# falfab/orb_slam_cuda

Measured on AMD Instinct MI355X. Metric: frames/s ORB extract+match, 1241×376 mono nFeatures=2000; achieved HBM GB/s, higher is better.
Workload: dtype u8

## Files before the change

orb_slam_cuda_amd/csrc/orbx_blur.hip:

```cpp
#include "orbx_device.cuh"

namespace orbx {

#ifndef ORBX_BLUR_TH
#define ORBX_BLUR_TH 48
#endif
#ifndef ORBX_BLUR_TW
#define ORBX_BLUR_TW 128
#endif
constexpr int kBlurTWs = 64, kBlurTHs = 32;

typedef unsigned short us2_t __attribute__((ext_vector_type(2)));
__device__ __forceinline__ uint32_t dot4(uint32_t px, uint32_t taps, uint32_t acc) {
  return __builtin_amdgcn_udot4(px, taps, acc, false);
}
__device__ __forceinline__ uint32_t dot2(uint32_t pair, uint32_t taps, uint32_t acc) {
  return __builtin_amdgcn_udot2(__builtin_bit_cast(us2_t, pair), __builtin_bit_cast(us2_t, taps), acc, false);
}

template <int kBlurTW, int kBlurTH>
__global__ __launch_bounds__(256) void blur_kernel(ExtractParams P, LevelPtrs lp, const int2* __restrict__ rtab,
                                                   int tiles, int ntiles, unsigned magic, uint8_t* __restrict__ blur) {
  constexpr int kBlurInW = kBlurTW + 32;
  constexpr int kBlurPairs = (kBlurTH + 6 + 1) / 2;
  __shared__ __attribute__((aligned(16))) uint8_t in[kBlurPairs * 2][kBlurInW];
  __shared__ __attribute__((aligned(16))) uint32_t tmp[kBlurPairs][kBlurTW];
  const int wg = xcd_remap(blockIdx.x + blockIdx.y * gridDim.x, gridDim.x * gridDim.y);
  const int f = magic ? (int)__umulhi((unsigned)wg, magic) : wg / ntiles, tid = threadIdx.x;
  const int e = rtab[tiles + wg - f * ntiles].x;
  const int l = e & 15, x0 = (e >> 4) & 0xFFF, y0 = e >> 16;
  const LevelGeom& g = P.lv[l];
  const int W = g.w, H = g.h;
  const uint8_t* S = lp.base[l] + f * lp.fstride[l];
  const int pitch = lp.pitch[l];
  typedef unsigned int u32x4 __attribute__((ext_vector_type(4)));
  constexpr int kChunks = kBlurInW / 16, kItems = (kBlurTH + 6) * kChunks, kPer = (kItems + 255) / 256;
  if (lp.aligned16[l]) {
    const int xmax = min(pitch, (W + 15) & ~15) - 16;
    u32x4 v[kPer];
#pragma unroll
    for (int q = 0; q < kPer; ++q) {
      const int i = min(tid + 256 * q, kItems - 1);
      const int r = i / kChunks, ch = i - r * kChunks;
      const int gy = reflect101(min(max(y0 + r - 3, -(H - 1)), 2 * H - 2), H);
      const int gx = min(max(x0 - 16 + ch * 16, 0), xmax);
      v[q] = *(const u32x4*)(S + (long long)gy * pitch + gx);
    }
#pragma unroll
    for (int q = 0; q < kPer; ++q) {
      const int i = min(tid + 256 * q, kItems - 1);
      const int r = i / kChunks, ch = i - r * kChunks;
      *(u32x4*)&in[r][ch * 16] = v[q];
    }
    const bool left = x0 == 0, right = x0 + kBlurTW + 3 > W;
    if (left || right) {
      __syncthreads();
      for (int i = tid; i < (kBlurTH + 6) * 6; i += 256) {
        const int r = i / 6, kk = i - r * 6;
        int x = kk < 3 ? -1 - kk : W + kk - 3;
        if ((kk < 3 && !left) || (kk >= 3 && !right) || x - x0 + 16 >= kBlurInW) continue;
        in[r][x - x0 + 16] = in[r][reflect101(x, W) - x0 + 16];
      }
    }
  } else {
    u32x4 v[kPer];
    bool direct[kPer];
    int gys[kPer];
#pragma unroll
    for (int q = 0; q < kPer; ++q) {
      const int i = min(tid + 256 * q, kItems - 1);
      const int r = i / kChunks, ch = i - r * kChunks;
      gys[q] = reflect101(min(max(y0 + r - 3, -(H - 1)), 2 * H - 2), H);
      const int gx = x0 - 16 + ch * 16;
      const uint8_t* src = S + (long long)gys[q] * pitch + gx;
      direct[q] = gx >= 0 && gx + 16 <= W && (((uintptr_t)src) & 15) == 0;
      v[q] = *(const u32x4*)(direct[q] ? src : S);
    }
#pragma unroll
    for (int q = 0; q < kPer; ++q) {
      const int i = min(tid + 256 * q, kItems - 1);
      const int r = i / kChunks, ch = i - r * kChunks;
      *(u32x4*)&in[r][ch * 16] = v[q];
    }
#pragma unroll
    for (int q = 0; q < kPer; ++q) {
      if (direct[q]) continue;
      const int i = min(tid + 256 * q, kItems - 1);
      const int r = i / kChunks, ch = i - r * kChunks;
      const int gx = x0 - 16 + ch * 16;
      const uint8_t* src = S + (long long)gys[q] * pitch;
#pragma unroll
      for (int k = 0; k < 16; ++k) {
        const int xx = min(max(gx + k, -(W - 1)), 2 * W - 2);
        in[r][ch * 16 + k] = src[reflect101(xx, W)];
      }
    }
  }
  __syncthreads();
  const int* k = P.gauss;
  const uint32_t kA0 = (k[0] << 8) | (k[1] << 16) | (k[2] << 24), kB0 = k[3] | (k[4] << 8) | (k[5] << 16) | (k[6] << 24);
  const uint32_t kA1 = (k[0] << 16) | (k[1] << 24), kB1 = k[2] | (k[3] << 8) | (k[4] << 16) | (k[5] << 24), kC1 = k[6];
  const uint32_t kA2 = k[0] << 24, kB2 = k[1] | (k[2] << 8) | (k[3] << 16) | (k[4] << 24), kC2 = k[5] | (k[6] << 8);
  const uint32_t kB3 = k[0] | (k[1] << 8) | (k[2] << 16) | (k[3] << 24), kC3 = k[4] | (k[5] << 8) | (k[6] << 16);
  for (int i = tid; i < kBlurPairs * (kBlurTW / 4); i += 256) {
    const int pr = i / (kBlurTW / 4), x = (i - pr * (kBlurTW / 4)) * 4;
    uint32_t o[2][4];
#pragma unroll
    for (int h = 0; h < 2; ++h) {
      const uint32_t* row = (const uint32_t*)in[2 * pr + h];
      const uint32_t A = row[(x + 12) >> 2], B = row[(x + 16) >> 2], C = row[(x + 20) >> 2];
      o[h][0] = dot4(B, kB0, dot4(A, kA0, 0));
      o[h][1] = dot4(C, kC1, dot4(B, kB1, dot4(A, kA1, 0)));
      o[h][2] = dot4(C, kC2, dot4(B, kB2, dot4(A, kA2, 0)));
      o[h][3] = dot4(C, kC3, dot4(B, kB3, 0));
    }
    *(uint4*)&tmp[pr][x] = make_uint4(o[0][0] | (o[1][0] << 16), o[0][1] | (o[1][1] << 16),
                                      o[0][2] | (o[1][2] << 16), o[0][3] | (o[1][3] << 16));
  }
  __syncthreads();
  const uint32_t t01 = k[0] | (k[1] << 16), t23 = k[2] | (k[3] << 16), t45 = k[4] | (k[5] << 16), t6 = k[6];
  const uint32_t u0 = k[0] << 16, u12 = k[1] | (k[2] << 16), u34 = k[3] | (k[4] << 16), u56 = k[5] | (k[6] << 16);
  uint8_t* D = blur + g.off + f * g.plane;
  for (int i = tid; i < (kBlurTH / 2) * (kBlurTW / 4); i += 256) {
    const int rp = i / (kBlurTW / 4), cx = (i - rp * (kBlurTW / 4)) * 4;
    const uint4 q0 = *(const uint4*)&tmp[rp][cx], q1 = *(const uint4*)&tmp[rp + 1][cx];
    const uint4 q2 = *(const uint4*)&tmp[rp + 2][cx], q3 = *(const uint4*)&tmp[rp + 3][cx];
    const uint32_t P0[4] = {q0.x, q0.y, q0.z, q0.w}, P1[4] = {q1.x, q1.y, q1.z, q1.w};
    const uint32_t P2[4] = {q2.x, q2.y, q2.z, q2.w}, P3[4] = {q3.x, q3.y, q3.z, q3.w};
    int va[4], vb[4];
#pragma unroll
    for (int q = 0; q < 4; ++q) {
      const uint32_t a = dot2(P3[q], t6, dot2(P2[q], t45, dot2(P1[q], t23, dot2(P0[q], t01, 1u << 15))));
      const uint32_t b = dot2(P3[q], u56, dot2(P2[q], u34, dot2(P1[q], u12, dot2(P0[q], u0, 1u << 15))));
      va[q] = min((int)(a >> 16), 255);
      vb[q] = min((int)(b >> 16), 255);
    }
    const uint32_t pa = pack4_u8(va[0], va[1], va[2], va[3]), pb = pack4_u8(vb[0], vb[1], vb[2], vb[3]);
    const int x = x0 + cx;
#pragma unroll
    for (int h = 0; h < 2; ++h) {
      const int y = y0 + 2 * rp + h;
      if (y >= H) break;
      const uint32_t packed = h ? pb : pa;
      uint8_t* dst = D + (long long)y * g.pitch + x;
      if (x + 4 <= W) {
        *(uint32_t*)dst = packed;
      } else {
        for (int q = 0; q < 4 && x + q < W; ++q) dst[q] = (uint8_t)(packed >> (8 * q));
      }
    }
  }
}

void blur_tile_dims(int small, int* tw, int* th) {
  *tw = small ? kBlurTWs : ORBX_BLUR_TW;
  *th = small ? kBlurTHs : ORBX_BLUR_TH;
}

int launch_blur(const ExtractParams& P, const LevelPtrs& lp, const int2* rtab, uint8_t* blur, int batch,
                hipStream_t s) {
  static const int cus = [] {
    int dev = 0, n = 256;
    (void)hipGetDevice(&dev);
    (void)hipDeviceGetAttribute(&n, hipDeviceAttributeMultiprocessorCount, dev);
    return n;
  }();
  if ((long long)P.blur_ntiles[0] * batch >= 2ll * cus)
    hipLaunchKernelGGL((blur_kernel<ORBX_BLUR_TW, ORBX_BLUR_TH>), dim3(P.blur_ntiles[0], batch), dim3(256), 0, s, P,
                       lp, rtab, P.blur_tiles[0], P.blur_ntiles[0], P.blur_magic[0], blur);
  else
    hipLaunchKernelGGL((blur_kernel<kBlurTWs, kBlurTHs>), dim3(P.blur_ntiles[1], batch), dim3(256), 0, s, P, lp,
                       rtab, P.blur_tiles[1], P.blur_ntiles[1], P.blur_magic[1], blur);
  return hipGetLastError() == hipSuccess ? ORBX_OK : ORBX_EDEVICE;
}

}
```

orb_slam_cuda_amd/csrc/orbx_host.hip:

```cpp
#include <hip/hip_runtime.h>

#include <algorithm>
#include <atomic>
#include <chrono>
#include <condition_variable>
#include <cfloat>
#include <cstdarg>
#include <climits>
#include <cmath>
#include <cstdio>
#include <cstdlib>
#include <cstring>
#include <mutex>
#include <string>
#include <thread>
#include <vector>

#include "orbx_internal.h"
#include "orbx_sincosf.h"

namespace orbx {

__global__ __launch_bounds__(256) void copy2d_kernel(uint8_t* __restrict__ d, size_t dp, const uint8_t* __restrict__ s,
                                                     size_t sp, size_t w, size_t rows) {
// ... 90 lines not shown
  int warm_w = 0, warm_h = 0;
  int last_batch = 0;
  const uint8_t* last_frames = nullptr;
  size_t last_fpitch = 0, last_rstride = 0;
  bool timing = false;
  hipEvent_t ev[6] = {};
  void* user_ev[ORBX_STAGE_EVENTS] = {};
  bool has_user_ev = false;
  WsOrder ws;
  bool host_pyr = false;
  bool host_pyr_valid = false;
  void* h_pyr = nullptr;
  size_t h_pyr_bytes = 0;
  long long h_pyr_off[kMaxLevels] = {};
  hipStream_t pstream = nullptr;
  hipEvent_t pev[2] = {};
  std::vector<float> prof_t[4];
  char order[6] = {};
  std::mutex mu;
};

WsOrder* orbx::extractor_ws(orbx_handle h) { return h ? &h->ws : nullptr; }

static void compute_scales(orbx_extractor* h) {
  const orbx_config& c = h->cfg;
  const int L = c.nlevels;
  h->scale.assign(L, 1.f);
  h->sigma2.assign(L, 1.f);
  for (int i = 1; i < L; i++) {
    h->scale[i] = h->scale[i - 1] * c.scale_factor;
    h->sigma2[i] = h->scale[i] * h->scale[i];
  }
  h->inv_scale.resize(L);
  h->inv_sigma2.resize(L);
  for (int i = 0; i < L; i++) {
    h->inv_scale[i] = 1.0f / h->scale[i];
    h->inv_sigma2[i] = 1.0f / h->sigma2[i];
  }
  h->nfeat.assign(L, 0);
  const float factor = 1.0f / c.scale_factor;
  float nDesired = c.nfeatures * (1 - factor) / (1 - (float)pow((double)factor, (double)L));
  int sum = 0;
  for (int l = 0; l < L - 1; l++) {
    h->nfeat[l] = cv_round(nDesired);
    sum += h->nfeat[l];
    nDesired *= factor;
  }
  h->nfeat[L - 1] = std::max(c.nfeatures - sum, 0);
  const int HP = kHalfPatch;
  int v, v0;
  const int vmax = cv_floor(HP * sqrtf(2.f) / 2 + 1);
  const int vmin = (int)std::ceil(HP * sqrtf(2.f) / 2);
  const double hp2 = HP * HP;
  for (v = 0; v <= vmax; ++v) h->umax[v] = (int)lrint(sqrt(hp2 - v * v));
  for (v = HP, v0 = 0; v >= vmin; --v) {
    while (h->umax[v0] == h->umax[v0 + 1]) ++v0;
    h->umax[v] = v0;
    ++v0;
  }
  if (c.scale_mode == ORBX_SCALE_F) {
    for (int l = 0; l < L; ++l) {
      const unsigned vw = (unsigned)std::ceil(c.width * std::pow(0.8408964, l));
      h->scale[l] = ((float)c.width) / vw;
      h->inv_scale[l] = ((float)vw) / c.width;
    }
  }
}

static void gaussian7(int k[7]) {
  float cf[7];
  double sum = 0;
  for (int i = 0; i < 7; ++i) {
    const double x = i - 3.0;
    cf[i] = (float)std::exp(-0.5 / (2.0 * 2.0) * x * x);
    sum += cf[i];
  }
  sum = 1. / sum;
  for (int i = 0; i < 7; ++i) cf[i] = (float)(cf[i] * sum);
  for (int i = 0; i < 7; ++i) k[i] = cv_round(cf[i] * 256.f);
}

static void resize_tables(int sw, int sh, int dw, int dh, std::vector<int2>& xt, std::vector<int2>& yt,
                          int* xmax_out, int* area2x) {
  const double inv_sx = (double)dw / sw, inv_sy = (double)dh / sh;
  const double scale_x = 1. / inv_sx, scale_y = 1. / inv_sy;
  const int isx = (int)lrint(scale_x), isy = (int)lrint(scale_y);
  const bool fast = std::fabs(scale_x - isx) < DBL_EPSILON && std::fabs(scale_y - isy) < DBL_EPSILON;
  *area2x = (fast && isx == 2 && isy == 2) ? 1 : 0;
  xt.resize(dw);
  yt.resize(dh);
  int xmax = dw;
  for (int dx = 0; dx < dw; ++dx) {
    float fx = (float)((dx + 0.5) * scale_x - 0.5);
    int sx = cv_floor(fx);
    fx -= sx;
    if (sx < 0) { fx = 0; sx = 0; }
    if (sx + 1 >= sw) {
      xmax = std::min(xmax, dx);
      if (sx >= sw - 1) { fx = 0; sx = sw - 1; }
    }
    const int a0 = sat_short(cv_round((1.f - fx) * 2048)), a1 = sat_short(cv_round(fx * 2048));
    xt[dx] = make_int2(sx, (a0 & 0xFFFF) | (a1 << 16));
  }
  *xmax_out = xmax;
  auto clip = [](int x, int a, int b) { return x >= a ? (x < b ? x : b - 1) : a; };
  for (int dy = 0; dy < dh; ++dy) {
    float fy = (float)((dy + 0.5) * scale_y - 0.5);
    int sy = cv_floor(fy);
    fy -= sy;
    const int b0 = sat_short(cv_round((1.f - fy) * 2048)), b1 = sat_short(cv_round(fy * 2048));
    yt[dy] = make_int2(clip(sy, 0, sh) | (clip(sy + 1, 0, sh) << 16), (b0 & 0xFFFF) | (b1 << 16));
  }
}

struct PyrCols {
  int nct = 1;
  std::vector<int> lo, chi, ohi;
  int lpitch[kMaxLevels] = {};
};

static bool plan_pyr_cols(const ExtractParams& P, const std::vector<int2>& rtab, int nct, PyrCols& C) {
  const int L = P.L, WL = P.lv[L - 1].w;
  if (nct > 1 && WL / nct < 32) return false;
  C.nct = nct;
  C.lo.assign((size_t)nct * L, 0);
  C.chi.assign((size_t)nct * L, 0);
  C.ohi.assign((size_t)nct * L, 0);
  auto src_lo_x = [&](int l, int x) { return rtab[P.lv[l].xtab2 + std::min(x, P.lv[l].w - 1)].x; };
  auto src_hi_x = [&](int l, int x) { return rtab[P.lv[l].xtab2 + std::min(x, P.lv[l].w - 1)].x + 1; };
  for (int c = 0; c < nct; ++c) {
    C.lo[c * L + L - 1] = c == 0 ? 0 : ((int)((long long)c * WL / nct) & ~1);
    C.chi[c * L + L - 1] = C.ohi[c * L + L - 1] = (c + 1 < nct ? ((int)((long long)(c + 1) * WL / nct) & ~1) : WL) - 1;
  }
  for (int l = L - 2; l >= 0; --l)
    for (int c = 0; c < nct; ++c) C.lo[c * L + l] = c == 0 ? 0 : (src_lo_x(l + 1, C.lo[c * L + l + 1]) & ~1);
  for (int l = L - 2; l >= 0; --l)
    for (int c = 0; c < nct; ++c) {
      const int own_hi = c + 1 < nct ? C.lo[(c + 1) * L + l] - 1 : P.lv[l].w - 1;
      if (own_hi < C.lo[c * L + l]) return false;
      C.ohi[c * L + l] = own_hi;
      C.chi[c * L + l] = std::max(src_hi_x(l + 1, C.chi[c * L + l + 1]), l > 0 ? own_hi : 0);
    }
  for (int l = 0; l < L; ++l) {
    int p = 0;
    for (int c = 0; c < nct; ++c) {
      const int lo = C.lo[c * L + l], hi = C.chi[c * L + l];
      p = std::max(p, l == 0 ? ((hi - (lo & ~15) + 1 + 15) & ~15) : ((hi - lo + 1 + 8 + 15) & ~15));
    }
    if (const char* e = getenv("ORBX_PYR_PADMOD")) {
      const int m = (l == 0 ? atoi(e) & ~15 : atoi(e)) % 128, step = l == 0 ? 16 : 4;
      while (p % 128 != m) p += step;
    }
    C.lpitch[l] = p;
  }
  return true;
}

static void plan_band_pyramid(ExtractParams& P, std::vector<int2>& rtab) {
  P.pyr_fused = 0;
  const int L = P.L;
  if (L < 2) return;
  auto src_lo = [&](int l, int y) { return P.lv[l].area2x ? 2 * y : (rtab[P.lv[l].ytab + y].x & 0xFFFF); };
  auto src_hi = [&](int l, int y) { return P.lv[l].area2x ? 2 * y + 1 : (rtab[P.lv[l].ytab + y].x >> 16); };
  const int HL = P.lv[L - 1].h;
  const size_t budgets[2] = {78 * 1024, 160 * 1024 - 1024};
  const int R0 = std::max(1, (HL + 17) / 18);
  struct Cand {
    int R, nb, nct;
    size_t need0, need1, ybytes;
    long long cost;
    std::vector<int> lo, chi, ohi;
    PyrCols cols;
  };
  std::vector<Cand> cands;
  PyrCols colplans[3];
  bool colok[3];
  for (int k = 0; k < 3; ++k) colok[k] = plan_pyr_cols(P, rtab, 1 << k, colplans[k]);
  const int Rmax = std::max(R0 + 5, (HL + 3) / 4);
  for (int R = Rmax; R >= std::max(1, R0 / 3); --R) {
    const int nb = (HL + R - 1) / R;
    if (!cands.empty() && cands.back().nb == nb) continue;
    std::vector<int> lo((size_t)nb * L), chi((size_t)nb * L), ohi((size_t)nb * L);
    for (int b = 0; b < nb; ++b) {
      lo[b * L + L - 1] = b * R;
      chi[b * L + L - 1] = ohi[b * L + L - 1] = std::min((b + 1) * R, HL) - 1;
    }
    for (int l = L - 2; l >= 0; --l)
      for (int b = 0; b < nb; ++b) lo[b * L + l] = b == 0 ? 0 : src_lo(l + 1, lo[b * L + l + 1]);
    for (int l = L - 2; l >= 0; --l)
      for (int b = 0; b < nb; ++b) {
        const int own_hi = b + 1 < nb ? lo[(b + 1) * L + l] - 1 : P.lv[l].h - 1;
        ohi[b * L + l] = own_hi;
        chi[b * L + l] = std::max(src_hi(l + 1, chi[b * L + l + 1]), l > 0 ? own_hi : 0);
      }
    size_t ybytes = 0;
    for (int b = 0; b < nb; ++b) {
      size_t s = 0;
      for (int l = 1; l < L; ++l) s += (size_t)(chi[b * L + l] - lo[b * L + l] + 1) * 8;
      ybytes = std::max(ybytes, s);
    }
    for (int k = 0; k < 3; ++k) {
      if (!colok[k]) continue;
      const PyrCols& C = colplans[k];
      size_t need[2] = {0, 0};
      for (int l = 0; l < L; ++l) {
        int rows = 0;
        for (int b = 0; b < nb; ++b) rows = std::max(rows, chi[b * L + l] - lo[b * L + l] + 1);
        need[l & 1] = std::max(need[l & 1], (size_t)rows * C.lpitch[l]);
      }
      need[0] = (need[0] + 15) & ~(size_t)15;
      need[1] = (need[1] + 15) & ~(size_t)15;
      if (need[0] + need[1] + ybytes + 16 > budgets[1]) continue;
      long long cost = 0;
      for (int b = 0; b < nb; ++b)
        for (int c = 0; c < C.nct; ++c) {
          long long s = 0;
          for (int l = 0; l < L; ++l)
            s += (long long)(chi[b * L + l] - lo[b * L + l] + 1) * (C.chi[c * L + l] - C.lo[c * L + l] + 1);
          cost = std::max(cost, s);
        }
      cands.push_back(Cand{R, nb, C.nct, need[0], need[1], ybytes, cost, lo, chi, ohi, C});
    }
  }
  if (cands.empty()) return;
  std::vector<int> keep;
  const char* ek = getenv("ORBX_PYR_KEEP");
  if (ek) {
    for (const char* p = ek; *p && keep.size() < 8;) {
      int nb = 0, nct = 0, used = 0;
      if (sscanf(p, "%d:%d%n", &nb, &nct, &used) != 2) break;
      for (int i = 0; i < (int)cands.size(); ++i)
        if (cands[i].nb == nb && cands[i].nct == nct) keep.push_back(i);
      p += used;
      if (*p == ',') ++p;
    }
  }
  if (keep.empty()) {
    int def = -1;
    for (int i = 0; i < (int)cands.size(); ++i)
      if (cands[i].nct == 1 && cands[i].need0 + cands[i].need1 + cands[i].ybytes + 16 <= budgets[0] &&
          (def < 0 || std::abs(cands[i].nb - (HL + R0 - 1) / R0) < std::abs(cands[def].nb - (HL + R0 - 1) / R0)))
        def = i;
    if (def < 0) def = 0;
    keep.push_back(def);
    std::vector<ExtractParams::PyrPlan> sim(cands.size());
    for (size_t i = 0; i < cands.size(); ++i) {
      sim[i].nbands = cands[i].nb;
      sim[i].nct = cands[i].nct;
      sim[i].cost = (int)cands[i].cost;
      sim[i].occ = cands[i].need0 + cands[i].need1 + cands[i].ybytes + 16 <= budgets[0] ? 2 : 1;
    }
    const int batches[8] = {1, 2, 4, 8, 16, 32, 64, P.B};
    for (int bt : batches) {
      const int best = pick_pyr_plan(sim.data(), (int)sim.size(), bt, 256);
      if (keep.size() < 8 && std::find(keep.begin(), keep.end(), best) == keep.end()) keep.push_back(best);
    }
    for (int d = 1; keep.size() < 8 && d < (int)cands.size(); ++d)
      for (int i : {def - d, def + d})
        if (i >= 0 && i < (int)cands.size() && cands[i].nct == 1 && keep.size() < 8 &&
            std::find(keep.begin(), keep.end(), i) == keep.end())
          keep.push_back(i);
  }
  P.pyr_nplans = 0;
  for (int i : keep) {
    const Cand& c = cands[i];
    ExtractParams::PyrPlan& q = P.pyr_plan[P.pyr_nplans++];
    q.nbands = c.nb;
    q.nct = c.nct;
    q.lds_a = (int)c.need0;
    q.lds_b = (int)c.need1;
    q.lds_y = (int)c.ybytes;
    q.cost = (int)c.cost;
    q.occ = 0;
    q.bands = (int)rtab.size();
    for (int b = 0; b < c.nb; ++b)
      for (int l = 0; l < L; ++l) {
        rtab.push_back(make_int2(c.lo[b * L + l], c.chi[b * L + l]));
        rtab.push_back(make_int2(c.lo[b * L + l], c.ohi[b * L + l]));
      }
    q.ctiles = (int)rtab.size();
    const PyrCols& C = c.cols;
    for (int t = 0; t < C.nct; ++t)
      for (int l = 0; l < L; ++l) {
        const int lo = C.lo[t * L + l];
        rtab.push_back(make_int2(lo, C.chi[t * L + l]));
        rtab.push_back(make_int2(lo, C.ohi[t * L + l]));
        rtab.push_back(make_int2(C.lpitch[l], l == 0 ? (lo & ~15) : lo));
      }
  }
  P.pyr_fused = 1;
  select_pyr_plan(P, 0);
}

static bool qt_code_tables(const LevelGeom& g, std::vector<uint32_t>& t, int* bits) {
  int R = 0;
  while ((1 << R) < g.nIni) ++R;
  if (R > 5 || g.boxW < 1 || g.boxH < 1 || g.boxW > 0xFFFF || g.boxH > 0xFFFF) return false;
  const int Dh = (13 - R) / 2;
  t.assign((size_t)g.boxW + g.boxH, 0u);
  for (int x = 0; x < g.boxW; ++x) {
    const int r = std::min((int)((float)x / g.hX), g.nIni - 1);
    int a = (int)(g.hX * (float)r), c = (int)(g.hX * (float)(r + 1));
    uint32_t code = (uint32_t)r << (2 * Dh);
    for (int j = 0; j < Dh; ++j) {
      const int mid = a + (int)std::ceil((float)(c - a) / 2.f);
      const int bit = x >= mid;
// ... 1091 lines not shown
```

orb_slam_cuda_amd/csrc/orbx_pyramid.hip:

```cpp
#include <cstdio>
#include <cstdlib>
#include <vector>

#include "orbx_device.cuh"

namespace orbx {

constexpr int kPyrTW = 256, kPyrTH = 16;
constexpr int kPyrMaxSrcW = 576;
constexpr int kPyrMaxSrcH = 36;

__global__ __launch_bounds__(256) void pyr_resize_kernel(
    const uint8_t* __restrict__ src, long long src_fs, int src_pitch, int sw, int sh, uint8_t* __restrict__ dst,
    long long dst_fs, int dst_pitch, int dw, int dh, const int2* __restrict__ xtab, const int2* __restrict__ ytab,
    int xmax, int area2x, int src_aligned16) {
  __shared__ __attribute__((aligned(16))) uint8_t tile[kPyrMaxSrcH][kPyrMaxSrcW];
  __shared__ int2 s_xt[kPyrTW];
  __shared__ int2 s_yt[kPyrTH];
  const int wg = xcd_remap(blockIdx.x + gridDim.x * (blockIdx.y + gridDim.y * blockIdx.z),
                           gridDim.x * gridDim.y * gridDim.z);
  const int f = wg / (gridDim.x * gridDim.y), tid = threadIdx.x;
  const int x0 = (wg % gridDim.x) * kPyrTW, y0 = ((wg / gridDim.x) % gridDim.y) * kPyrTH;
  const int nx = min(kPyrTW, dw - x0), ny = min(kPyrTH, dh - y0);
  const uint8_t* S = src + f * src_fs;
  int sx_lo, sx_hi, sy_lo, sy_hi;
  if (area2x) {
    if (tid < nx) s_xt[tid] = make_int2(2 * (x0 + tid), 0);
    if (tid < ny) s_yt[tid] = make_int2(2 * (y0 + tid) | ((2 * (y0 + tid) + 1) << 16), 0);
    sx_lo = 2 * x0;
    sx_hi = 2 * (x0 + nx - 1) + 1;
    sy_lo = 2 * y0;
    sy_hi = 2 * (y0 + ny - 1) + 1;
  } else {
    if (tid < nx) s_xt[tid] = xtab[x0 + tid];
    if (tid < ny) s_yt[tid] = ytab[y0 + tid];
    sx_lo = xtab[x0].x;
    sx_hi = min(xtab[x0 + nx - 1].x + 1, sw - 1);
    sy_lo = ytab[y0].x & 0xFFFF;
    sy_hi = ytab[y0 + ny - 1].x >> 16;
  }
  const int a0 = src_aligned16 ? (sx_lo & ~15) : sx_lo;
  const int nrow = sy_hi - sy_lo + 1;
  if (src_aligned16) {
    const int nch = (sx_hi - a0 + 16) >> 4;
    for (int i = tid; i < nrow * nch; i += 256) {
      const int r = i / nch, ch = i - r * nch;
      const uint8_t* g = S + (long long)(sy_lo + r) * src_pitch + a0 + ch * 16;
      if (a0 + ch * 16 + 16 <= src_pitch) {
        *(uint4*)&tile[r][ch * 16] = *(const uint4*)g;
      } else {
        for (int k = 0; k < 16 && a0 + ch * 16 + k < sw; ++k) tile[r][ch * 16 + k] = g[k];
      }
    }
  } else {
    const int ncol = sx_hi - a0 + 1;
    for (int i = tid; i < nrow * ncol; i += 256) {
      const int r = i / ncol, c = i - r * ncol;
      tile[r][c] = S[(long long)(sy_lo + r) * src_pitch + a0 + c];
    }
  }
  __syncthreads();
  const int cx = (tid & 63) * 4, ry = (tid >> 6) * 4;
  if (cx >= nx) return;
  int sxl[4], a0v[4], a1v[4], rep[4];
#pragma unroll
  for (int q = 0; q < 4; ++q) {
    const int c = min(cx + q, nx - 1);
    const int2 xt = s_xt[c];
    sxl[q] = xt.x - a0;
    a0v[q] = (short)(xt.y & 0xFFFF);
    a1v[q] = (short)(xt.y >> 16);
    rep[q] = area2x ? 0 : (x0 + c >= xmax);
  }
  uint8_t* D = dst + f * dst_fs + (long long)(y0 + ry) * dst_pitch + x0 + cx;
#pragma unroll
  for (int rr = 0; rr < 4; ++rr) {
    if (ry + rr >= ny) break;
    const int2 yt = s_yt[ry + rr];
    const uint8_t* r0 = tile[(yt.x & 0xFFFF) - sy_lo];
    const uint8_t* r1 = tile[(yt.x >> 16) - sy_lo];
    int v[4];
#pragma unroll
    for (int q = 0; q < 4; ++q) {
      const int s = sxl[q];
      if (area2x) {
        v[q] = (r0[s] + r0[s + 1] + r1[s] + r1[s + 1] + 2) >> 2;
      } else {
        int D0, D1;
        if (!rep[q]) {
          D0 = __mul24((int)r0[s], a0v[q]) + __mul24((int)r0[s + 1], a1v[q]);
          D1 = __mul24((int)r1[s], a0v[q]) + __mul24((int)r1[s + 1], a1v[q]);
        } else {
          D0 = r0[s] * 2048;
          D1 = r1[s] * 2048;
        }
        const int b0 = (short)(yt.y & 0xFFFF), b1 = (short)(yt.y >> 16);
        v[q] = sat_u8((__mul24(D0, b0) + __mul24(D1, b1) + (1 << 21)) >> 22);
      }
    }
    const uint32_t packed = pack4_u8(v[0], v[1], v[2], v[3]);
    uint8_t* drow = D + (long long)rr * dst_pitch;
    if (cx + 4 <= nx) {
      *(uint32_t*)drow = packed;
    } else {
      for (int q = 0; cx + q < nx; ++q) drow[q] = (uint8_t)(packed >> (8 * q));
    }
  }
}

#ifndef ORBX_PYR_THREADS
#define ORBX_PYR_THREADS 512
#endif
constexpr int kPyrBandThreads = ORBX_PYR_THREADS;
#ifndef ORBX_PYR_WPE
#define ORBX_PYR_WPE 5
#endif

#ifndef ORBX_PYR_RUN
#define ORBX_PYR_RUN 2
#endif
#ifndef ORBX_PYR_ROWFAST
#define ORBX_PYR_ROWFAST 0
#endif
constexpr int kPyrRun = ORBX_PYR_RUN, kPyrRuns = 8 / kPyrRun;
static_assert(kPyrRun == 2 || kPyrRun == 4, "runs of 2 or 4 columns");
__device__ __forceinline__ int pyr_col(int gi, int G, int q) { return kPyrRun * (gi + (q / kPyrRun) * G) + q % kPyrRun; }

template <bool AREA2X>
__device__ __forceinline__ void band_rows(const LevelPtrs& lp, int l, int f, const uint8_t* src, int spitch,
                                          uint8_t* dst, int dpitch, const int2* yt_rows, int src_lo, int2 cd,
                                          int2 own, int2 ownx, int x0, int r0, int rstep, int gi, int G,
                                          const int (&sx)[8], const int (&a0v)[8], const int (&a1v)[8]) {
  uint8_t* G0 = (uint8_t*)lp.base[l] + f * lp.fstride[l];
  for (int r = cd.x + r0; r <= cd.y; r += rstep) {
    const int2 yt = yt_rows[r - cd.x];
    const uint8_t* s0 = src + __mul24((yt.x & 0xFFFF) - src_lo, spitch);
    const uint8_t* s1 = src + __mul24((yt.x >> 16) - src_lo, spitch);
    int p00[8], p01[8], p10[8], p11[8];
#pragma unroll
    for (int q = 0; q < 8; ++q) {
      p00[q] = s0[sx[q]];
      p01[q] = s0[sx[q] + 1];
      p10[q] = s1[sx[q]];
      p11[q] = s1[sx[q] + 1];
    }
    int v[8];
    if (AREA2X) {
#pragma unroll
      for (int q = 0; q < 8; ++q) v[q] = (p00[q] + p01[q] + p10[q] + p11[q] + 2) >> 2;
    } else {
      const int b0 = (short)(yt.y & 0xFFFF), b1 = (short)(yt.y >> 16);
#pragma unroll
      for (int q = 0; q < 8; ++q) {
        const int D0 = __mul24(p00[q], a0v[q]) + __mul24(p01[q], a1v[q]);
        const int D1 = __mul24(p10[q], a0v[q]) + __mul24(p11[q], a1v[q]);
        v[q] = sat_u8((__mul24(D0, b0) + __mul24(D1, b1) + (1 << 21)) >> 22);
      }
    }
    uint8_t* lrow = dst + __mul24(r - cd.x, dpitch);
    const bool owned = r >= own.x && r <= own.y;
    uint8_t* drow = G0 + (long long)r * lp.pitch[l];
    if constexpr (kPyrRun == 4) {
      const int xa = pyr_col(gi, G, 0), xb = pyr_col(gi, G, 4);
      const uint32_t pa = pack4_u8(v[0], v[1], v[2], v[3]), pb = pack4_u8(v[4], v[5], v[6], v[7]);
      *(uint32_t*)(lrow + xa) = pa;
      *(uint32_t*)(lrow + xb) = pb;
      if (owned) {
        for (int q = 0; q < 4; ++q) {
          const int ga = x0 + xa + q, gb = x0 + xb + q;
          if (ga >= ownx.x && ga <= ownx.y) drow[ga] = (uint8_t)(pa >> (8 * q));
          if (gb >= ownx.x && gb <= ownx.y) drow[gb] = (uint8_t)(pb >> (8 * q));
        }
      }
    } else {
#pragma unroll
      for (int k = 0; k < kPyrRuns; ++k) {
        const int xk = pyr_col(gi, G, 2 * k);
        const uint16_t pk = (uint16_t)(sat_u8(v[2 * k]) | (sat_u8(v[2 * k + 1]) << 8));
        *(uint16_t*)(lrow + xk) = pk;
        const int gx = x0 + xk;
        if (owned && gx >= ownx.x && gx <= ownx.y) {
          if (gx < ownx.y) *(uint16_t*)(drow + gx) = pk;
          else drow[gx] = (uint8_t)pk;
        }
      }
    }
  }
}

__global__ __launch_bounds__(kPyrBandThreads) __attribute__((amdgpu_waves_per_eu(ORBX_PYR_WPE))) void pyr_band_kernel(ExtractParams P, LevelPtrs lp,
                                                                   const int2* __restrict__ rtab, int* dbg) {
  extern __shared__ __attribute__((aligned(16))) uint8_t smem[];
  const unsigned long long t_begin = __builtin_amdgcn_s_memtime();
  const int nb = P.pyr_nbands, nct = P.pyr_nct, L = P.L, tid = threadIdx.x;
  const int wg = xcd_remap(blockIdx.x, gridDim.x);
  const int f = wg / (nb * nct), tile = wg - f * (nb * nct), band = tile / nct, ct = tile - band * nct;
  const int2* bt = rtab + P.pyr_bands + (long long)band * L * 2;
  const int2* xt = rtab + P.pyr_ctiles + (long long)ct * L * 3;
  uint8_t* const bufA = smem;
  uint8_t* const bufB = smem + P.pyr_lds_a;
  int2* const s_yt = (int2*)(smem + P.pyr_lds_a + P.pyr_lds_b);
  int yrow = 0, ytot = 0, yarea = 1, ytab = 0;
#pragma unroll
  for (int l = 1; l < kMaxLevels; ++l) {
    const int2 cd = bt[2 * min(l, L - 1)];
    const int n = l < L ? cd.y - cd.x + 1 : 0;
    if (tid >= ytot && tid < ytot + n) {
      yrow = cd.x + tid - ytot;
      yarea = P.lv[l].area2x;
      ytab = P.lv[l].ytab;
    }
    ytot += n;
  }
  int2 yval = make_int2(0, 0);
  if (tid < ytot) yval = yarea ? make_int2((2 * yrow) | ((2 * yrow + 1) << 16), 0) : rtab[ytab + yrow];
  for (int i = tid + kPyrBandThreads; i < ytot; i += kPyrBandThreads) {
    int rem = i;
    for (int l = 1; l < L; ++l) {
      const int2 cd = bt[2 * l];
      const int n = cd.y - cd.x + 1;
      if (rem < n) {
        const LevelGeom& g = P.lv[l];
        const int r = cd.x + rem;
        s_yt[i] = g.area2x ? make_int2((2 * r) | ((2 * r + 1) << 16), 0) : rtab[g.ytab + r];
        break;
      }
      rem -= n;
    }
  }

  {
    const int2 c0 = bt[0], x0c = xt[0], x0p = xt[2];
    const int rows = c0.y - c0.x + 1, lp0 = x0p.x, org = x0p.y, pitch = lp.pitch[0];
    const int xe = min(x0c.y, P.lv[0].w - 1);
    const uint8_t* S = lp.base[0] + f * lp.fstride[0] + (long long)c0.x * pitch + org;
    if (lp.aligned16[0]) {
      typedef unsigned int u32x4 __attribute__((ext_vector_type(4)));
      const int nch = ((xe - org) >> 4) + 1, total = rows * nch;
      for (int i0 = tid; i0 < total; i0 += 4 * kPyrBandThreads) {
        u32x4 v[4];
        int so[4], lo[4];
#pragma unroll
        for (int q = 0; q < 4; ++q) {
          const int i = min(i0 + q * kPyrBandThreads, total - 1);
          const int r = i / nch, ch = i - r * nch;
          lo[q] = r * pitch + ch * 16;
          so[q] = r * lp0 + ch * 16;
        }
#pragma unroll
        for (int q = 0; q < 4; ++q) v[q] = *(const u32x4*)(S + lo[q]);
        if (i0 == tid && tid < ytot) s_yt[tid] = yval;
#pragma unroll
        for (int q = 0; q < 4; ++q) *(u32x4*)(bufA + so[q]) = v[q];
      }
      if (tid >= total && tid < ytot) s_yt[tid] = yval;
    } else {
      if (tid < ytot) s_yt[tid] = yval;
      const int ncol = xe - org + 1;
      for (int r = 0; r < rows; ++r)
        for (int c = tid; c < ncol; c += kPyrBandThreads) bufA[r * lp0 + c] = S[(long long)r * pitch + c];
    }
  }

  int2 nxt[8];
  auto fetch_cols = [&](int l) {
    const LevelGeom& g = P.lv[l];
    const int2 xc = xt[3 * l];
#if ORBX_PYR_ROWFAST
    const int G = (xc.y - xc.x + 1 + 7) >> 3, gi = min(tid / (kPyrBandThreads / G), G - 1);
#else
    const int G = (xc.y - xc.x + 1 + 7) >> 3, gi = tid % G;
#endif
#pragma unroll
    for (int q = 0; q < 8; ++q) nxt[q] = rtab[g.xtab2 + min(xc.x + pyr_col(gi, G, q), g.w - 1)];
  };
  fetch_cols(1);
  lds_sync();
  if (dbg && tid == 0) dbg[blockIdx.x * 16] = (int)(__builtin_amdgcn_s_memtime() - t_begin);

  int yoff = 0;
  for (int l = 1; l < L; ++l) {
    const LevelGeom& g = P.lv[l];
    const uint8_t* src = (l & 1) ? bufA : bufB;
    uint8_t* dst = (l & 1) ? bufB : bufA;
    const int2 cs = bt[2 * (l - 1)], cd = bt[2 * l], own = bt[2 * l + 1];
    const int2 xc = xt[3 * l], xo = xt[3 * l + 1], sp = xt[3 * (l - 1) + 2], dp = xt[3 * l + 2];
    const int G = (xc.y - xc.x + 1 + 7) >> 3, rstep = kPyrBandThreads / G;
#if ORBX_PYR_ROWFAST
    const int gi = tid / rstep, r0 = tid < rstep * G ? tid - gi * rstep : rstep;
#else
    const int gi = tid % G, r0 = tid / G;
#endif
    int sx[8], a0v[8], a1v[8];
#pragma unroll
    for (int q = 0; q < 8; ++q) {
      sx[q] = nxt[q].x - sp.y;
      a0v[q] = (short)(nxt[q].y & 0xFFFF);
      a1v[q] = (short)(nxt[q].y >> 16);
    }
    if (l + 1 < L) fetch_cols(l + 1);
    if (r0 < rstep) {
      if (g.area2x)
        band_rows<true>(lp, l, f, src, sp.x, dst, dp.x, s_yt + yoff, cs.x, cd, own, xo, xc.x, r0, rstep, gi, G, sx,
                        a0v, a1v);
      else
        band_rows<false>(lp, l, f, src, sp.x, dst, dp.x, s_yt + yoff, cs.x, cd, own, xo, xc.x, r0, rstep, gi, G, sx,
                         a0v, a1v);
    }
    yoff += cd.y - cd.x + 1;
    lds_sync();
    if (dbg && tid == 0) dbg[blockIdx.x * 16 + l] = (int)(__builtin_amdgcn_s_memtime() - t_begin);
  }
}

size_t pyr_band_lds_bytes(const ExtractParams& P) { return (size_t)P.pyr_lds_a + P.pyr_lds_b + P.pyr_lds_y + 16; }
const void* pyr_band_kernel_ptr() { return (const void*)pyr_band_kernel; }
int pyr_band_occupancy(size_t lds) {
  int n = 0;
  if (hipOccupancyMaxActiveBlocksPerMultiprocessor(&n, pyr_band_kernel, kPyrBandThreads, lds) != hipSuccess) return 1;
  return std::max(1, n);
}

static int launch_band(const ExtractParams& P, const LevelPtrs& lp, const int2* rtab, int batch, hipStream_t s) {
  static int* dbg = nullptr;
  static int dbg_cap = 0;
  static const bool prof = getenv("ORBX_PYR_PROF") && getenv("ORBX_PYR_PROF")[0] == '1';
  const int nwg = P.pyr_nbands * P.pyr_nct * batch;
  if (prof && nwg > dbg_cap) {
    if (dbg) (void)hipFree(dbg);
    (void)hipMalloc(&dbg, (size_t)nwg * 16 * 4);
    dbg_cap = nwg;
  }
  hipLaunchKernelGGL(pyr_band_kernel, dim3(nwg), dim3(kPyrBandThreads), pyr_band_lds_bytes(P), s, P, lp, rtab,
                     prof ? dbg : nullptr);
  if (prof) {
    std::vector<int> h((size_t)nwg * 16);
    (void)hipStreamSynchronize(s);
    (void)hipMemcpy(h.data(), dbg, h.size() * 4, hipMemcpyDeviceToHost);
    double avg[16] = {0};
    int mx[16] = {0};
    for (int w = 0; w < nwg; ++w)
      for (int k = 0; k < P.L; ++k) {
        avg[k] += h[w * 16 + k];
        mx[k] = std::max(mx[k], h[w * 16 + k]);
      }
    fprintf(stderr, "pyr_band plans (bands x tiles/cost/lds):");
    for (int i = 0; i < P.pyr_nplans; ++i)
      fprintf(stderr, " %dx%d/%d/%d", P.pyr_plan[i].nbands, P.pyr_plan[i].nct, P.pyr_plan[i].cost,
              P.pyr_plan[i].lds_a + P.pyr_plan[i].lds_b + P.pyr_plan[i].lds_y + 16);
    fprintf(stderr, "\n");
    fprintf(stderr, "pyr_band: %d WGs (%d bands x %d tiles); phase cycles avg/max:", nwg, P.pyr_nbands, P.pyr_nct);
    for (int k = 0; k < P.L; ++k) fprintf(stderr, " [%d] %.0f/%d", k, avg[k] / nwg, mx[k]);
    fprintf(stderr, "\n");
  }
  return hipGetLastError() == hipSuccess ? ORBX_OK : ORBX_EDEVICE;
}

int launch_pyramid(const ExtractParams& P, const LevelPtrs& lp, const int2* rtab, int batch, hipStream_t s) {
  if (P.L < 2) return ORBX_OK;
  if (P.pyr_fused) {
    static const int cus = [] {
      int dev = 0, n = 256;
      (void)hipGetDevice(&dev);
      (void)hipDeviceGetAttribute(&n, hipDeviceAttributeMultiprocessorCount, dev);
      return n;
    }();
    const char* fp = getenv("ORBX_PYR_PLAN");
    const int forced = fp ? atoi(fp) : -1;
    ExtractParams Q = P;
    select_pyr_plan(Q, forced >= 0 && forced < P.pyr_nplans
                           ? forced
                           : pick_pyr_plan(P, batch, cus));
    return launch_band(Q, lp, rtab, batch, s);
  }
  for (int l = 1; l < P.L; ++l) {
    const LevelGeom& sg = P.lv[l - 1];
    const LevelGeom& d = P.lv[l];
    dim3 grid((d.w + kPyrTW - 1) / kPyrTW, (d.h + kPyrTH - 1) / kPyrTH, batch);
    hipLaunchKernelGGL(pyr_resize_kernel, grid, dim3(256), 0, s, lp.base[l - 1], lp.fstride[l - 1], lp.pitch[l - 1],
                       sg.w, sg.h, (uint8_t*)lp.base[l], lp.fstride[l], lp.pitch[l], d.w, d.h, rtab + d.xtab,
                       rtab + d.ytab, d.xmax, d.area2x, lp.aligned16[l - 1]);
  }
  return hipGetLastError() == hipSuccess ? ORBX_OK : ORBX_EDEVICE;
}

}
```

Before: 180,000.

## Restructure pyramid band resize to contiguous row chunks with reuse and dot2 filtering

The band pyramid kernel now gives each thread a contiguous run of output rows instead of striding, so a horizontally filtered source row shared between consecutive output rows can be reused. Pixel loads become dword loads with byte permutes, the horizontal pass uses udot2 and the vertical pass uses 24-bit multiply-add. Integer divides are replaced with float-reciprocal divides. The blur kernel also skips horizontal and vertical work for rows beyond the image bottom, and the host adds a config check that rejects layouts the new dword loads cannot handle. Risks are float-division rounding errors and weight-scaling changes that could alter the output.

Measured after the change: 183,300 (median of 6 runs). 1.02x the previous value.

```diff
diff --git a/orb_slam_cuda_amd/csrc/orbx_blur.hip b/orb_slam_cuda_amd/csrc/orbx_blur.hip
--- a/orb_slam_cuda_amd/csrc/orbx_blur.hip
+++ b/orb_slam_cuda_amd/csrc/orbx_blur.hip
@@ -102,7 +102,8 @@
   const uint32_t kA1 = (k[0] << 16) | (k[1] << 24), kB1 = k[2] | (k[3] << 8) | (k[4] << 16) | (k[5] << 24), kC1 = k[6];
   const uint32_t kA2 = k[0] << 24, kB2 = k[1] | (k[2] << 8) | (k[3] << 16) | (k[4] << 24), kC2 = k[5] | (k[6] << 8);
   const uint32_t kB3 = k[0] | (k[1] << 8) | (k[2] << 16) | (k[3] << 24), kC3 = k[4] | (k[5] << 8) | (k[6] << 16);
-  for (int i = tid; i < kBlurPairs * (kBlurTW / 4); i += 256) {
+  const int opairs = (min(kBlurTH, H - y0) + 1) >> 1;
+  for (int i = tid; i < min(kBlurPairs, opairs + 3) * (kBlurTW / 4); i += 256) {
     const int pr = i / (kBlurTW / 4), x = (i - pr * (kBlurTW / 4)) * 4;
     uint32_t o[2][4];
 #pragma unroll
@@ -121,7 +122,7 @@
   const uint32_t t01 = k[0] | (k[1] << 16), t23 = k[2] | (k[3] << 16), t45 = k[4] | (k[5] << 16), t6 = k[6];
   const uint32_t u0 = k[0] << 16, u12 = k[1] | (k[2] << 16), u34 = k[3] | (k[4] << 16), u56 = k[5] | (k[6] << 16);
   uint8_t* D = blur + g.off + f * g.plane;
-  for (int i = tid; i < (kBlurTH / 2) * (kBlurTW / 4); i += 256) {
+  for (int i = tid; i < opairs * (kBlurTW / 4); i += 256) {
     const int rp = i / (kBlurTW / 4), cx = (i - rp * (kBlurTW / 4)) * 4;
     const uint4 q0 = *(const uint4*)&tmp[rp][cx], q1 = *(const uint4*)&tmp[rp + 1][cx];
     const uint4 q2 = *(const uint4*)&tmp[rp + 2][cx], q3 = *(const uint4*)&tmp[rp + 3][cx];
diff --git a/orb_slam_cuda_amd/csrc/orbx_host.hip b/orb_slam_cuda_amd/csrc/orbx_host.hip
--- a/orb_slam_cuda_amd/csrc/orbx_host.hip
+++ b/orb_slam_cuda_amd/csrc/orbx_host.hip
@@ -266,6 +266,11 @@
       while (p % 128 != m) p += step;
     }
     C.lpitch[l] = p;
+  }
+  for (int l = 1; l < L; ++l) {
+    if (C.lpitch[l - 1] % 4) return false;
+    for (int c = 0; c < nct; ++c)
+      if (C.chi[c * L + l] - C.lo[c * L + l] + 1 > 8 * 512) return false;
   }
   return true;
 }
diff --git a/orb_slam_cuda_amd/csrc/orbx_pyramid.hip b/orb_slam_cuda_amd/csrc/orbx_pyramid.hip
--- a/orb_slam_cuda_amd/csrc/orbx_pyramid.hip
+++ b/orb_slam_cuda_amd/csrc/orbx_pyramid.hip
@@ -112,79 +112,85 @@
 #define ORBX_PYR_THREADS 512
 #endif
 constexpr int kPyrBandThreads = ORBX_PYR_THREADS;
+constexpr uint32_t kPyrAreaA = 2048u | (2048u << 16);
+constexpr int kPyrAreaB4 = 2048 | (2048 << 16);
 #ifndef ORBX_PYR_WPE
 #define ORBX_PYR_WPE 5
 #endif
 
-#ifndef ORBX_PYR_RUN
-#define ORBX_PYR_RUN 2
-#endif
-#ifndef ORBX_PYR_ROWFAST
-#define ORBX_PYR_ROWFAST 0
-#endif
-constexpr int kPyrRun = ORBX_PYR_RUN, kPyrRuns = 8 / kPyrRun;
-static_assert(kPyrRun == 2 || kPyrRun == 4, "runs of 2 or 4 columns");
-__device__ __forceinline__ int pyr_col(int gi, int G, int q) { return kPyrRun * (gi + (q / kPyrRun) * G) + q % kPyrRun; }
-
-template <bool AREA2X>
-__device__ __forceinline__ void band_rows(const LevelPtrs& lp, int l, int f, const uint8_t* src, int spitch,
-                                          uint8_t* dst, int dpitch, const int2* yt_rows, int src_lo, int2 cd,
-                                          int2 own, int2 ownx, int x0, int r0, int rstep, int gi, int G,
-                                          const int (&sx)[8], const int (&a0v)[8], const int (&a1v)[8]) {
-  uint8_t* G0 = (uint8_t*)lp.base[l] + f * lp.fstride[l];
-  for (int r = cd.x + r0; r <= cd.y; r += rstep) {
-    const int2 yt = yt_rows[r - cd.x];
-    const uint8_t* s0 = src + __mul24((yt.x & 0xFFFF) - src_lo, spitch);
-    const uint8_t* s1 = src + __mul24((yt.x >> 16) - src_lo, spitch);
-    int p00[8], p01[8], p10[8], p11[8];
-#pragma unroll
-    for (int q = 0; q < 8; ++q) {
-      p00[q] = s0[sx[q]];
-      p01[q] = s0[sx[q] + 1];
-      p10[q] = s1[sx[q]];
-      p11[q] = s1[sx[q] + 1];
-    }
-    int v[8];
-    if (AREA2X) {
-#pragma unroll
-      for (int q = 0; q < 8; ++q) v[q] = (p00[q] + p01[q] + p10[q] + p11[q] + 2) >> 2;
-    } else {
-      const int b0 = (short)(yt.y & 0xFFFF), b1 = (short)(yt.y >> 16);
-#pragma unroll
-      for (int q = 0; q < 8; ++q) {
-        const int D0 = __mul24(p00[q], a0v[q]) + __mul24(p01[q], a1v[q]);
-        const int D1 = __mul24(p10[q], a0v[q]) + __mul24(p11[q], a1v[q]);
-        v[q] = sat_u8((__mul24(D0, b0) + __mul24(D1, b1) + (1 << 21)) >> 22);
-      }
-    }
-    uint8_t* lrow = dst + __mul24(r - cd.x, dpitch);
-    const bool owned = r >= own.x && r <= own.y;
-    uint8_t* drow = G0 + (long long)r * lp.pitch[l];
-    if constexpr (kPyrRun == 4) {
-      const int xa = pyr_col(gi, G, 0), xb = pyr_col(gi, G, 4);
-      const uint32_t pa = pack4_u8(v[0], v[1], v[2], v[3]), pb = pack4_u8(v[4], v[5], v[6], v[7]);
-      *(uint32_t*)(lrow + xa) = pa;
-      *(uint32_t*)(lrow + xb) = pb;
-      if (owned) {
-        for (int q = 0; q < 4; ++q) {
-          const int ga = x0 + xa + q, gb = x0 + xb + q;
-          if (ga >= ownx.x && ga <= ownx.y) drow[ga] = (uint8_t)(pa >> (8 * q));
-          if (gb >= ownx.x && gb <= ownx.y) drow[gb] = (uint8_t)(pb >> (8 * q));
-        }
-      }
-    } else {
-#pragma unroll
-      for (int k = 0; k < kPyrRuns; ++k) {
-        const int xk = pyr_col(gi, G, 2 * k);
-        const uint16_t pk = (uint16_t)(sat_u8(v[2 * k]) | (sat_u8(v[2 * k + 1]) << 8));
-        *(uint16_t*)(lrow + xk) = pk;
-        const int gx = x0 + xk;
-        if (owned && gx >= ownx.x && gx <= ownx.y) {
-          if (gx < ownx.y) *(uint16_t*)(drow + gx) = pk;
-          else drow[gx] = (uint8_t)pk;
-        }
-      }
-    }
+__device__ __forceinline__ int pyr_col(int gi, int G, int q) { return 2 * (gi + (q >> 1) * G) + (q & 1); }
+
+typedef unsigned short pyr_us2_t __attribute__((ext_vector_type(2)));
+
+__device__ __forceinline__ int band_div(int i, float rcp) { return (int)(((float)i + 0.5f) * rcp); }
+
+struct BandCols {
+  int off[4];
+  uint32_t sel[8];
+  uint32_t a01[8];
+};
+__device__ __forceinline__ void band_load(const uint8_t* row, const BandCols& bc, uint32_t (&p)[8]) {
+#pragma unroll
+  for (int k = 0; k < 4; ++k) {
+    const uint32_t* d = (const uint32_t*)(row + bc.off[k]);
+    p[2 * k] = d[0];
+    p[2 * k + 1] = d[1];
+  }
+}
+__device__ __forceinline__ void band_hpass(const uint32_t (&p)[8], const BandCols& bc, uint32_t (&D)[8]) {
+#pragma unroll
+  for (int q = 0; q < 8; ++q) {
+    const uint32_t pp = __builtin_amdgcn_perm(p[q | 1], p[q & ~1], bc.sel[q]);
+    D[q] = __builtin_amdgcn_udot2(__builtin_bit_cast(pyr_us2_t, pp), __builtin_bit_cast(pyr_us2_t, bc.a01[q]), 0u, false);
+  }
+}
+
+__device__ __forceinline__ uint32_t band_mad24(uint32_t a, uint32_t b, uint32_t c) {
+  uint32_t d;
+  asm("v_mad_u32_u24 %0, %1, %2, %3" : "=v"(d) : "v"(a), "v"(b), "v"(c));
+  return d;
+}
+
+struct BandRowCtx {
+  const uint8_t* src;
+  uint8_t* dst;
+  uint8_t* g[4];
+  const int2* yt;
+  int spitch, dpitch, gpitch, src_lo, row0;
+  unsigned own_lo, own_n;
+  bool st2[4], st1[4], any1;
+};
+__device__ __forceinline__ void band_row(const BandRowCtx& c, int r, uint32_t loff, uint32_t goff, int& have,
+                                         const BandCols& bc, int G, uint32_t (&Da)[8], uint32_t (&Db)[8]) {
+  const int2 yt = c.yt[r - c.row0];
+  const int y0 = yt.x & 0xFFFF, y1 = yt.x >> 16;
+  const uint8_t* const row1 = c.src + __mul24(y1 - c.src_lo, c.spitch);
+  uint32_t p1[8];
+  if (y0 != have) {
+    uint32_t p0[8];
+    band_load(c.src + __mul24(y0 - c.src_lo, c.spitch), bc, p0);
+    band_load(row1, bc, p1);
+    band_hpass(p0, bc, Da);
+  } else {
+    band_load(row1, bc, p1);
+  }
+  band_hpass(p1, bc, Db);
+  have = y1;
+  const uint32_t b0 = (uint32_t)yt.y & 0xFFFFu, b1 = (uint32_t)yt.y >> 16;
+  const bool owned = (unsigned)r - c.own_lo < c.own_n;
+  uint32_t pk[4];
+#pragma unroll
+  for (int k = 0; k < 4; ++k) {
+    const uint32_t va = band_mad24(Da[2 * k], b0, band_mad24(Db[2 * k], b1, 1u << 23));
+    const uint32_t vb = band_mad24(Da[2 * k + 1], b0, band_mad24(Db[2 * k + 1], b1, 1u << 23));
+    pk[k] = __builtin_amdgcn_perm(vb, va, 0x0c0c0703u);
+    *(uint16_t*)(c.dst + loff + 2 * k * G) = (uint16_t)pk[k];
+    if (owned && c.st2[k]) *(uint16_t*)(c.g[k] + goff) = (uint16_t)pk[k];
+  }
+  if (c.any1 && owned) {
+#pragma unroll
+    for (int k = 0; k < 4; ++k)
+      if (c.st1[k]) c.g[k][goff] = (uint8_t)pk[k];
   }
 }
 
@@ -212,8 +218,13 @@
     }
     ytot += n;
   }
+  auto y_entry = [&](int area, int tab, int r) {
+    if (area) return make_int2((2 * r) | ((2 * r + 1) << 16), kPyrAreaB4);
+    const int2 e = rtab[tab + r];
+    return make_int2(e.x, e.y << 2);
+  };
   int2 yval = make_int2(0, 0);
-  if (tid < ytot) yval = yarea ? make_int2((2 * yrow) | ((2 * yrow + 1) << 16), 0) : rtab[ytab + yrow];
+  if (tid < ytot) yval = y_entry(yarea, ytab, yrow);
   for (int i = tid + kPyrBandThreads; i < ytot; i += kPyrBandThreads) {
     int rem = i;
     for (int l = 1; l < L; ++l) {
@@ -222,7 +233,7 @@
       if (rem < n) {
         const LevelGeom& g = P.lv[l];
         const int r = cd.x + rem;
-        s_yt[i] = g.area2x ? make_int2((2 * r) | ((2 * r + 1) << 16), 0) : rtab[g.ytab + r];
+        s_yt[i] = y_entry(g.area2x, g.ytab, r);
         break;
       }
       rem -= n;
@@ -237,13 +248,14 @@
     if (lp.aligned16[0]) {
       typedef unsigned int u32x4 __attribute__((ext_vector_type(4)));
       const int nch = ((xe - org) >> 4) + 1, total = rows * nch;
+      const float rnch = __builtin_amdgcn_rcpf((float)nch);
       for (int i0 = tid; i0 < total; i0 += 4 * kPyrBandThreads) {
         u32x4 v[4];
         int so[4], lo[4];
 #pragma unroll
         for (int q = 0; q < 4; ++q) {
           const int i = min(i0 + q * kPyrBandThreads, total - 1);
-          const int r = i / nch, ch = i - r * nch;
+          const int r = band_div(i, rnch), ch = i - r * nch;
           lo[q] = r * pitch + ch * 16;
           so[q] = r * lp0 + ch * 16;
         }
@@ -263,14 +275,19 @@
   }
 
   int2 nxt[8];
+  int nxt_gi = 0, nxt_ra = 0, nxt_rb = -1;
   auto fetch_cols = [&](int l) {
     const LevelGeom& g = P.lv[l];
     const int2 xc = xt[3 * l];
-#if ORBX_PYR_ROWFAST
-    const int G = (xc.y - xc.x + 1 + 7) >> 3, gi = min(tid / (kPyrBandThreads / G), G - 1);
-#else
-    const int G = (xc.y - xc.x + 1 + 7) >> 3, gi = tid % G;
-#endif
+    const int G = (xc.y - xc.x + 1 + 7) >> 3;
+    const float rG = __builtin_amdgcn_rcpf((float)G);
+    const int chunk = band_div(tid, rG), gi = tid - chunk * G;
+    const int2 cd = bt[2 * l];
+    const int nrows = cd.y - cd.x + 1, nchunks = band_div(kPyrBandThreads, rG);
+    const int len = band_div(nrows, __builtin_amdgcn_rcpf((float)nchunks)), rem = nrows - len * nchunks;
+    nxt_gi = gi;
+    nxt_ra = cd.x + chunk * len + min(chunk, rem);
+    nxt_rb = chunk < nchunks ? nxt_ra + len - (chunk < rem ? 0 : 1) : nxt_ra - 1;
 #pragma unroll
     for (int q = 0; q < 8; ++q) nxt[q] = rtab[g.xtab2 + min(xc.x + pyr_col(gi, G, q), g.w - 1)];
   };
@@ -281,31 +298,42 @@
   int yoff = 0;
   for (int l = 1; l < L; ++l) {
     const LevelGeom& g = P.lv[l];
-    const uint8_t* src = (l & 1) ? bufA : bufB;
-    uint8_t* dst = (l & 1) ? bufB : bufA;
     const int2 cs = bt[2 * (l - 1)], cd = bt[2 * l], own = bt[2 * l + 1];
     const int2 xc = xt[3 * l], xo = xt[3 * l + 1], sp = xt[3 * (l - 1) + 2], dp = xt[3 * l + 2];
-    const int G = (xc.y - xc.x + 1 + 7) >> 3, rstep = kPyrBandThreads / G;
-#if ORBX_PYR_ROWFAST
-    const int gi = tid / rstep, r0 = tid < rstep * G ? tid - gi * rstep : rstep;
-#else
-    const int gi = tid % G, r0 = tid / G;
-#endif
-    int sx[8], a0v[8], a1v[8];
+    const int G = (xc.y - xc.x + 1 + 7) >> 3, gi = nxt_gi, ra = nxt_ra, rb = nxt_rb;
+    BandCols bc;
 #pragma unroll
     for (int q = 0; q < 8; ++q) {
-      sx[q] = nxt[q].x - sp.y;
-      a0v[q] = (short)(nxt[q].y & 0xFFFF);
-      a1v[q] = (short)(nxt[q].y >> 16);
+      const int sx = nxt[q].x - sp.y;
+      if (!(q & 1)) bc.off[q >> 1] = sx & ~3;
+      const uint32_t o = (uint32_t)(sx - bc.off[q >> 1]);
+      bc.sel[q] = 0x0c000c00u | o | ((o + 1) << 16);
+      bc.a01[q] = g.area2x ? kPyrAreaA : (uint32_t)nxt[q].y;
     }
     if (l + 1 < L) fetch_cols(l + 1);
-    if (r0 < rstep) {
-      if (g.area2x)
-        band_rows<true>(lp, l, f, src, sp.x, dst, dp.x, s_yt + yoff, cs.x, cd, own, xo, xc.x, r0, rstep, gi, G, sx,
-                        a0v, a1v);
-      else
-        band_rows<false>(lp, l, f, src, sp.x, dst, dp.x, s_yt + yoff, cs.x, cd, own, xo, xc.x, r0, rstep, gi, G, sx,
-                         a0v, a1v);
+    BandRowCtx c;
+    c.src = (l & 1) ? bufA : bufB;
+    c.dst = (l & 1) ? bufB : bufA;
+    c.yt = s_yt + yoff;
+    c.spitch = sp.x, c.dpitch = dp.x, c.gpitch = lp.pitch[l], c.src_lo = cs.x, c.row0 = cd.x;
+    c.own_lo = (unsigned)own.x, c.own_n = (unsigned)(own.y - own.x + 1);
+#pragma unroll
+    for (int k = 0; k < 4; ++k) {
+      const int gx = xc.x + 2 * (gi + k * G);
+      c.g[k] = (uint8_t*)lp.base[l] + f * lp.fstride[l] + xc.x + 2 * k * G;
+      c.st2[k] = gx >= xo.x && gx < xo.y;
+      c.st1[k] = gx == xo.y;
+    }
+    c.any1 = c.st1[0] | c.st1[1] | c.st1[2] | c.st1[3];
+    uint32_t loff = (uint32_t)(__mul24(ra - cd.x, c.dpitch) + 2 * gi);
+    uint32_t goff = (uint32_t)(ra * c.gpitch + 2 * gi);
+    uint32_t Da[8], Db[8];
+    int have = -1;
+    for (int r = ra; r <= rb; r += 2) {
+      band_row(c, r, loff, goff, have, bc, G, Da, Db);
+      loff += c.dpitch, goff += c.gpitch;
+      if (r + 1 <= rb) band_row(c, r + 1, loff, goff, have, bc, G, Db, Da);
+      loff += c.dpitch, goff += c.gpitch;
     }
     yoff += cd.y - cd.x + 1;
     lds_sync();
```
